# sarpel/wakeword-jupyterlab

Measured on AMD Instinct MI355X. Metric: 1s/16kHz clips/sec end-to-end (mel+CNN+LSTM), higher is better.
Workload: dtype f32 in/out/accumulate; conv and LSTM-gate GEMM products as f16x3 split (3 f16 MFMAs per fp32 product block, ~2^-21 rel.)

## Files before the change

### wakeword-jupyterlab_amd/csrc/ww_logmel.hip

```cpp
#include <mutex>
#include <type_traits>

#include "ww_internal.h"

namespace ww {

constexpr int kSlab = 2048 + 4;
constexpr int kPartialInSlab = 1032;
static_assert(kPartialInSlab + kPieces <= kSlab, "piece sums must fit behind the power spectrum");

template <int WAVES, int FR = kFrames>
struct K1Layout {
    static constexpr int kWaves = WAVES;
    static constexpr int kThreads = WAVES * 64;
    static constexpr int kMelStr = FR + 1;
    static constexpr int kOffMel = WAVES * kSlab;
    static constexpr int kOffRed = kOffMel + kMels * kMelStr;
    static constexpr int kOffFrm = kOffRed + 16;
    static constexpr int kOffInvw = kOffFrm + WAVES * FR;
    static constexpr int kOffFlag = kOffInvw + kMels;
    static constexpr int kOffDcNy = kOffFlag + 4;
    static constexpr int kOffPinfo = kOffDcNy + FR;
    static constexpr int kOffFp0 = kOffPinfo + kPieces;
    static constexpr int kOffFcnt = kOffFp0 + kMels;
    static constexpr int kOffTw2 = kOffFcnt + kMels;
    static constexpr int kOffTwp = kOffTw2 + 7 * 16 * 2;
    static constexpr int kLdsFloats = kOffTwp + 512 * 2;
    static constexpr int kWavesPerSimd = WAVES == 4 ? (FR != kFrames ? 2 : 3) : 2;
    static constexpr int kBlocksPerCu = WAVES == 4 ? (FR != kFrames ? 2 : 3) : 1;
    static_assert(kOffPinfo % 4 == 0 && kOffTw2 % 4 == 0 && kOffTwp % 2 == 0, "LDS table alignment");
    static_assert(FR % WAVES == 0 && WAVES <= 8, "frames are dealt to the waves in whole rounds; red[] holds 16 floats");
    static_assert(FR == kFrames || FR == 64, "the long-clip tile: 64 frames, frames dealt round-robin");
    static_assert(kBlocksPerCu * sizeof(float) * kLdsFloats <= 160 * 1024, "LDS per CU");
};

__device__ __forceinline__ float2 operator+(float2 a, float2 b) { return make_float2(a.x + b.x, a.y + b.y); }
__device__ __forceinline__ float2 operator-(float2 a, float2 b) { return make_float2(a.x - b.x, a.y - b.y); }
__device__ __forceinline__ float2 cmul(float2 a, float2 b) {
    return make_float2(fmaf(a.x, b.x, -a.y * b.y), fmaf(a.x, b.y, a.y * b.x));
}
__device__ __forceinline__ float2 mul_neg_i(float2 a) { return make_float2(a.y, -a.x); }

__device__ __forceinline__ void dft4(float2& a0, float2& a1, float2& a2, float2& a3) {
    const float2 t0 = a0 + a2, t1 = a0 - a2, t2 = a1 + a3, t3 = mul_neg_i(a1 - a3);
    a0 = t0 + t2; a2 = t0 - t2; a1 = t1 + t3; a3 = t1 - t3;
}

__device__ __forceinline__ void dft8(float2 (&v)[8]) {
    constexpr float c = 0.70710678118654752440f;
    float2 e0 = v[0], e1 = v[2], e2 = v[4], e3 = v[6];
    float2 o0 = v[1], o1 = v[3], o2 = v[5], o3 = v[7];
    dft4(e0, e1, e2, e3);
    dft4(o0, o1, o2, o3);
    o1 = make_float2(c * (o1.x + o1.y), c * (o1.y - o1.x));
    o2 = mul_neg_i(o2);
    o3 = make_float2(c * (o3.y - o3.x), -c * (o3.x + o3.y));
    v[0] = e0 + o0; v[4] = e0 - o0;
    v[1] = e1 + o1; v[5] = e1 - o1;
    v[2] = e2 + o2; v[6] = e2 - o2;
    v[3] = e3 + o3; v[7] = e3 - o3;
}

__device__ __forceinline__ void dft16(float2 (&v)[16]) {
    float2 e[8], o[8];
#pragma unroll
    for (int i = 0; i < 8; ++i) { e[i] = v[2 * i]; o[i] = v[2 * i + 1]; }
    dft8(e);
    dft8(o);
    constexpr float c1 = 0.92387953251128675613f, s1 = 0.38268343236508977173f;
    constexpr float c2 = 0.70710678118654752440f;
    const float2 w[8] = {{1.f, 0.f}, {c1, -s1}, {c2, -c2}, {s1, -c1}, {0.f, -1.f}, {-s1, -c1}, {-c2, -c2}, {-c1, -s1}};
#pragma unroll
    for (int k = 0; k < 8; ++k) {
        const float2 t = (k == 0) ? o[0] : (k == 4 ? mul_neg_i(o[4]) : cmul(o[k], w[k]));
        v[k] = e[k] + t;
        v[k + 8] = e[k] - t;
    }
}

__device__ __forceinline__ float db10(float x) {
#pragma clang fp contract(off)
    return 10.0f * log10f(x);
}

__device__ __forceinline__ void lds_order() {
    __builtin_amdgcn_fence(__ATOMIC_RELEASE, "wavefront");
    __builtin_amdgcn_wave_barrier();
    __builtin_amdgcn_fence(__ATOMIC_ACQUIRE, "wavefront");
}

__device__ __forceinline__ float absmax3(float a, float b, float m) {
    float r;
    asm("v_max3_f32 %0, |%1|, |%2|, %3" : "=v"(r) : "v"(a), "v"(b), "v"(m));
    return r;
}

using u32x4_t = __attribute__((ext_vector_type(4))) unsigned int;

template <bool RING>
__device__ __forceinline__ void load_frame(float4 (&sn)[8], __amdgpu_buffer_rsrc_t rsrc, int base, int ring_pos, int ring_len) {
#pragma unroll
    for (int n1 = 0; n1 < 8; ++n1) {
        const int idx = base + 256 * n1;
        int off = idx * 4;
        if constexpr (RING) {
            int at = idx + ring_pos;
            at = at >= ring_len ? at - ring_len : at;
            off = (idx >= 0 && idx < ring_len) ? at * 4 : -1;
        }
        const u32x4_t v = __builtin_amdgcn_raw_buffer_load_b128(rsrc, off, 0, 0);
        sn[n1] = __builtin_bit_cast(float4, v);
    }
}

constexpr uint32_t kRedoMark = 0x7fc5a11eu;
constexpr float kFloorRatio = 1.0e-5f;

#ifdef WW_STAMPS
__device__ unsigned long long g_stamps[16];
#define STAMP(i) do { unsigned long long t__; asm volatile("s_memtime %0\n\ts_waitcnt lgkmcnt(0)" : "=s"(t__) :: "memory"); \
    if (stamp_on) { acc_st[i] += t__ - last_st; } last_st = t__; } while (0)
#else
#define STAMP(i) do {} while (0)
#endif

template <bool RING, int WAVES, int FR = kFrames>
__global__ __launch_bounds__(WAVES * 64, (K1Layout<WAVES, FR>::kWavesPerSimd)) void logmel_kernel(const float* __restrict__ pcm, int64_t clip_stride,
                                                             int clip_len, int n_clips, int normalize,
                                                             const int32_t* __restrict__ ring_pos_p, int ring_len,
                                                             const LogmelTables* __restrict__ tb,
                                                             float* __restrict__ out, int mark, int n_frames) {
    using L = K1Layout<WAVES, FR>;
    constexpr int kMelStride = L::kMelStr;
    const int nfr = FR == kFrames ? kFrames : n_frames;
    constexpr int kWavesPerBlock = WAVES, kThreads = L::kThreads;
    constexpr int kOffMel = L::kOffMel, kOffRed = L::kOffRed, kOffFrm = L::kOffFrm, kOffInvw = L::kOffInvw, kOffFlag = L::kOffFlag,
                  kOffDcNy = L::kOffDcNy, kOffPinfo = L::kOffPinfo, kOffFp0 = L::kOffFp0,
                  kOffFcnt = L::kOffFcnt, kOffTw2 = L::kOffTw2, kOffTwp = L::kOffTwp;
    extern __shared__ __attribute__((aligned(16))) float lds[];
    float* mel = lds + kOffMel;
    float* red = lds + kOffRed;
    const float4* pw4 = reinterpret_cast<const float4*>(&tb->piece_w[0][0][0]);
    const int* pinfo = reinterpret_cast<const int*>(lds + kOffPinfo);
    const int* fp0 = reinterpret_cast<const int*>(lds + kOffFp0);
    const int* fcnt = reinterpret_cast<const int*>(lds + kOffFcnt);
    const float4* tw2_4 = reinterpret_cast<const float4*>(lds + kOffTw2);
    const float2* twp_2 = reinterpret_cast<const float2*>(lds + kOffTwp);

    const int tid = threadIdx.x;
    const int lane_id = tid & 63;
    const int lane = lane_id;
    const int wave = __builtin_amdgcn_readfirstlane(tid >> 6);
    float* slab = lds + wave * kSlab;
    float2* slab2 = reinterpret_cast<float2*>(slab);
    float4* slab4 = reinterpret_cast<float4*>(slab);
    float* partial = slab + kPartialInSlab;
    const float4* tw1_4 = reinterpret_cast<const float4*>(&tb->tw1[0][0]);
    const float4* win4 = reinterpret_cast<const float4*>(&tb->window[0]);

    for (int i = tid; i < kPieces; i += kThreads) reinterpret_cast<int*>(lds)[kOffPinfo + i] = tb->piece_info[i];
    if (tid < kMels) {
        reinterpret_cast<int*>(lds)[kOffFp0 + tid] = tb->filt_p0[tid];
        reinterpret_cast<int*>(lds)[kOffFcnt + tid] = tb->filt_cnt[tid];
        lds[kOffInvw + tid] = tb->band_bins[tid];
    }
    if (tid < 4) reinterpret_cast<uint32_t*>(lds)[kOffFlag + tid] = 0u;
    for (int i = tid; i < 7 * 16 * 2; i += kThreads) lds[kOffTw2 + i] = (&tb->tw2[0][0].x)[i];
    for (int i = tid; i < 512 * 2; i += kThreads) lds[kOffTwp + i] = (&tb->twp[0].x)[i];
    const int ring_pos = RING ? *ring_pos_p : 0;
    __syncthreads();
    const int my_p0a = fp0[lane], my_cnta = fcnt[lane];
    const int my_p0b = lane + 64 < kMels ? fp0[lane + 64] : 0, my_cntb = lane + 64 < kMels ? fcnt[lane + 64] : 0;

#ifdef WW_STAMPS
    const bool stamp_on = true;
    unsigned long long acc_st[10] = {0, 0, 0, 0, 0, 0, 0, 0, 0, 0}, last_st = 0;
    STAMP(9);
#endif

    const unsigned clip_bytes = unsigned(clip_len) * 4u;
    auto clip_rsrc = [&](int c) {
        const bool ok = c < n_clips;
        const float* base = pcm + int64_t(ok ? c : 0) * clip_stride;
        return __builtin_amdgcn_make_buffer_rsrc(const_cast<float*>(base), 0, ok ? clip_bytes : 0u, 0x00020000);
    };
    const int kRounds = FR == kFrames ? kFrames / kWavesPerBlock : (nfr + kWavesPerBlock - 1) / kWavesPerBlock;
    const int frame0 = wave;
    float4 sn[8];
    load_frame<RING>(sn, clip_rsrc(blockIdx.x), frame0 * kHop - kNfft / 2 + 4 * lane, ring_pos, ring_len);
    int clip_it = 0;
#pragma unroll 1
    for (int clip = blockIdx.x; clip < n_clips; clip += gridDim.x, ++clip_it) {
        const __amdgpu_buffer_rsrc_t rs_cur = clip_rsrc(clip), rs_next = clip_rsrc(clip + int(gridDim.x));
        float peak = 0.f;

#pragma unroll 1
        for (int round = 0; round < kRounds; ++round) {
            const int frame = round * kWavesPerBlock + wave;
            int lane = lane_id;
            asm volatile("" : "+v"(lane));
            const int k1r = lane >> 3, jr = lane & 7;
            const int base_next = (frame + kWavesPerBlock) * kHop - kNfft / 2 + 4 * lane;

            STAMP(8);
            float2 za[8], zb[8];
#pragma unroll
            for (int n1 = 0; n1 < 8; ++n1) {
                const float4 s = sn[n1];
                const float4 w = win4[64 * n1 + lane];
                if (n1 == 4 || n1 == 5) peak = absmax3(s.z, s.w, absmax3(s.x, s.y, peak));
                za[n1] = make_float2(s.x * w.x, s.y * w.y);
                zb[n1] = make_float2(s.z * w.z, s.w * w.w);
            }
            float4 t1[7];
#pragma unroll
            for (int k1 = 1; k1 < 8; ++k1) t1[k1 - 1] = tw1_4[(k1 - 1) * 64 + lane];
            __builtin_amdgcn_sched_barrier(0);
            dft8(za);
            dft8(zb);
            slab4[lane] = make_float4(za[0].x, za[0].y, zb[0].x, zb[0].y);
#pragma unroll
            for (int k1 = 1; k1 < 8; ++k1) {
                const float4 t = t1[k1 - 1];
                const float2 a = cmul(za[k1], make_float2(t.x, t.y));
                const float2 b = cmul(zb[k1], make_float2(t.z, t.w));
                slab4[k1 * 64 + (lane ^ (8 * ((k1 >> 1) & 1)))] = make_float4(a.x, a.y, b.x, b.y);
            }
            lds_order();
            STAMP(0);
            {
                const int s8 = 8 * ((k1r >> 1) & 1);
                const float4* x1e = slab4 + k1r * 64 + jr + s8;
                const float4* x1o = slab4 + k1r * 64 + jr - s8;
#pragma unroll
                for (int n2 = 0; n2 < 8; ++n2) {
                    const float4 v = (n2 & 1) ? x1o[n2 * 8] : x1e[n2 * 8];
                    za[n2] = make_float2(v.x, v.y);
                    zb[n2] = make_float2(v.z, v.w);
                }
                float4 t2[7];
#pragma unroll
                for (int k2 = 1; k2 < 8; ++k2) t2[k2 - 1] = tw2_4[(k2 - 1) * 8 + jr];
                lds_order();
                __builtin_amdgcn_sched_barrier(0);
                dft8(za);
                dft8(zb);
                float4* x2w[4];
#pragma unroll
                for (int hk = 0; hk < 4; ++hk) x2w[hk] = slab4 + 64 * k1r + (jr ^ (4 * (k1r & 1) + hk));
#pragma unroll
                for (int k2 = 0; k2 < 8; ++k2) {
                    float2 a = za[k2], b = zb[k2];
                    if (k2 > 0) {
                        const float4 t = t2[k2 - 1];
                        a = cmul(a, make_float2(t.x, t.y));
                        b = cmul(b, make_float2(t.z, t.w));
                    }
                    x2w[k2 >> 1][8 * k2] = make_float4(a.x, a.y, b.x, b.y);
                }
            }
            lds_order();
            STAMP(1);
            {
                float2 u[16];
                const int sw2 = (lane >> 1) & 7;
#pragma unroll
                for (int m = 0; m < 8; ++m) {
                    const float4 v = slab4[lane * 8 + (m ^ sw2)];
                    u[2 * m] = make_float2(v.x, v.y);
                    u[2 * m + 1] = make_float2(v.z, v.w);
                }
                lds_order();
                dft16(u);
                const int lp = (lane >> 3) + 8 * (lane & 7);
                float2* zw = slab2 + (lp ^ (((lp >> 4) & 3) << 1));
#pragma unroll
                for (int kk = 0; kk < 16; ++kk) zw[64 * kk] = u[kk];
            }
            lds_order();
            STAMP(2);
            float4 pw0[kPieceRounds], pw1[kPieceRounds];
#pragma unroll
            for (int c = 0; c < kPieceRounds; ++c) {
                pw0[c] = pw4[c * kPieceSlots + lane];
                pw1[c] = pw4[kPieces + c * kPieceSlots + lane];
            }
            {
                const bool last = round + 1 == kRounds;
                load_frame<RING>(sn, last ? rs_next : rs_cur, last ? frame0 * kHop - kNfft / 2 + 4 * lane : base_next, ring_pos,
                                 ring_len);
            }
            {
                float2 a[8], b[8];
                const int lowb = (64 - lane) & 63;
                const float2* za_p = slab2 + (lane ^ (((lane >> 4) & 3) << 1));
                const float2* zb_p = slab2 + (lowb ^ (((lowb >> 4) & 3) << 1)) + (lane == 0 ? 64 : 0);
#pragma unroll
                for (int j = 0; j < 8; ++j) {
                    a[j] = za_p[64 * j];
                    b[j] = zb_p[64 * (15 - j)];
                }
                if (lane == 0) {
                    if (mark) lds[kOffDcNy + frame] = 2.0f * fmaf(a[0].x, a[0].x, a[0].y * a[0].y);
                    a[0] = slab2[512];
                    b[0] = a[0];
                }
                float2 twj[8];
#pragma unroll
                for (int j = 0; j < 8; ++j) twj[j] = twp_2[lane + 64 * j];
                lds_order();
                __builtin_amdgcn_sched_barrier(0);
#pragma unroll
                for (int j = 0; j < 8; ++j) {
                    const int k = (j == 0 && lane == 0) ? 512 : lane + 64 * j;
                    const float2 tw = twj[j];
                    const float2 e = make_float2(0.5f * (a[j].x + b[j].x), 0.5f * (a[j].y - b[j].y));
                    const float2 o = make_float2(0.5f * (a[j].y + b[j].y), 0.5f * (b[j].x - a[j].x));
                    const float2 t = cmul(o, tw);
                    const float2 p = e + t, m = e - t;
                    slab[k] = fmaf(p.x, p.x, p.y * p.y);
                    slab[1024 - k] = fmaf(m.x, m.x, m.y * m.y);
                }
                if (lane == 0) slab[0] = 0.f;
            }
            lds_order();
            STAMP(3);
            {
                int info[kPieceRounds];
                float4 s0[kPieceRounds], s1[kPieceRounds];
#pragma unroll
                for (int c = 0; c < kPieceRounds; ++c) info[c] = pinfo[c * kPieceSlots + lane];
#pragma unroll
                for (int c = 0; c < kPieceRounds; ++c) {
                    const float4* s4 = reinterpret_cast<const float4*>(slab + (info[c] & 0xffff));
                    s0[c] = s4[0];
                    s1[c] = s4[1];
                }
                __builtin_amdgcn_sched_barrier(0);
#pragma unroll
                for (int c = 0; c < kPieceRounds; ++c) {
                    const float4 w0 = pw0[c], w1 = pw1[c];
                    float acc = w0.x * s0[c].x;
                    acc = fmaf(w0.y, s0[c].y, acc);
                    acc = fmaf(w0.z, s0[c].z, acc);
                    acc = fmaf(w0.w, s0[c].w, acc);
                    acc = fmaf(w1.x, s1[c].x, acc);
                    acc = fmaf(w1.y, s1[c].y, acc);
                    acc = fmaf(w1.z, s1[c].z, acc);
                    acc = fmaf(w1.w, s1[c].w, acc);
                    partial[info[c] >> 16] = acc;
                }
                lds_order();
                STAMP(4);
#pragma unroll
                for (int pass = 0; pass < 2; ++pass) {
                    const int f = lane + 64 * pass;
                    const int p0 = pass ? my_p0b : my_p0a, cnt = pass ? my_cntb : my_cnta;
                    if (f < kMels) {
                        float v[10];
#pragma unroll
                        for (int q = 0; q < 10; ++q) v[q] = partial[p0 + (q < cnt ? q : 0)];
                        float acc = 0.f;
#pragma unroll
                        for (int q = 0; q < 10; ++q) acc += (q < cnt) ? v[q] : 0.f;
                        mel[f * kMelStride + frame] = acc;
                    }
                }
            }
            lds_order();
            STAMP(5);
        }
        if constexpr (FR != kFrames) {
            __syncthreads();
            uint32_t* flag = reinterpret_cast<uint32_t*>(lds) + kOffFlag;
            if (mark && tid == 0) { flag[2 * ((clip_it + 1) & 1)] = 0u; flag[2 * ((clip_it + 1) & 1) + 1] = 0u; }
            const bool fr_live = lane < nfr;
            const float* invw = lds + kOffInvw;
            float* frm = lds + kOffFrm;
            float mmax = 0.f, e_part = 0.f;
            if (fr_live)
                for (int b = wave; b < kMels; b += kWavesPerBlock) {
                    const float p = mel[b * kMelStride + lane];
                    mmax = fmaxf(mmax, p);
                    if (mark) e_part = fmaf(p, invw[b], e_part);
                }
            if (mark) frm[wave * FR + lane] = e_part;
#pragma unroll
            for (int off = 32; off > 0; off >>= 1) {
                mmax = fmaxf(mmax, __shfl_xor(mmax, off));
                peak = fmaxf(peak, __shfl_xor(peak, off));
            }
            if (lane == 0) { red[wave] = mmax; red[kWavesPerBlock + wave] = peak; }
            __syncthreads();
            mmax = red[0];
            peak = red[kWavesPerBlock];
#pragma unroll
            for (int w = 1; w < kWavesPerBlock; ++w) { mmax = fmaxf(mmax, red[w]); peak = fmaxf(peak, red[kWavesPerBlock + w]); }
            const float amin = 1e-10f;
            float g2 = 1.f;
            if (normalize) { const float g = 1.0f / peak; g2 = g * g; }
            float ref = mmax * g2;
            ref = ref < amin ? amin : ref;
            const float ref_db = db10(ref);
            float* __restrict__ o = out + int64_t(clip) * (kMels * nfr);
            float floor_e = 0.f;
            if (mark) {
#pragma unroll
                for (int w = 0; w < kWavesPerBlock; ++w) floor_e += frm[w * FR + lane];
                floor_e += lds[kOffDcNy + lane];
                floor_e *= kFloorRatio;
            }
            const float live_thr = fmaxf(mmax * 0.99e-8f, amin / g2);
            bool redo = false;
            if (fr_live)
                for (int b = wave; b < kMels; b += kWavesPerBlock) {
                    const float p = mel[b * kMelStride + lane];
                    float v = p * g2;
                    v = v < amin ? amin : v;
                    float db = db10(v) - ref_db;
                    db = db < -80.0f ? -80.0f : db;
                    o[b * nfr + lane] = db;
                    if (mark) redo |= p > live_thr && p * invw[b] < floor_e;
                }
            if (mark) {
                const unsigned long long bal = __builtin_amdgcn_ballot_w64(redo);
                if (bal != 0ull && lane == 0) {
                    __hip_atomic_fetch_or(flag + 2 * (clip_it & 1), uint32_t(bal), __ATOMIC_RELAXED, __HIP_MEMORY_SCOPE_WORKGROUP);
                    __hip_atomic_fetch_or(flag + 2 * (clip_it & 1) + 1, uint32_t(bal >> 32), __ATOMIC_RELAXED, __HIP_MEMORY_SCOPE_WORKGROUP);
                }
            }
            __syncthreads();
            if (mark) {
                const uint32_t f_lo = flag[2 * (clip_it & 1)], f_hi = flag[2 * (clip_it & 1) + 1];
                if ((f_lo | f_hi) != 0u) {
                    if (fr_live)
                        for (int b = wave; b < kMels; b += kWavesPerBlock)
                            if (b * nfr + lane >= 3) o[b * nfr + lane] = mel[b * kMelStride + lane] * g2;
                    if (tid == 0) {
                        reinterpret_cast<uint32_t*>(o)[0] = kRedoMark;
                        reinterpret_cast<uint32_t*>(o)[1] = f_lo | 7u;
                        reinterpret_cast<uint32_t*>(o)[2] = f_hi;
                    }
                    __syncthreads();
                }
            }
        } else {
        __syncthreads();
        STAMP(6);
        uint32_t* flag = reinterpret_cast<uint32_t*>(lds) + kOffFlag;
        if (mark && tid == 0) flag[(clip_it + 1) & 1] = 0u;

        float mmax = 0.f, e_part = 0.f;
        const float* invw = lds + kOffInvw;
        float* frm = lds + kOffFrm;
        for (int idx = tid; idx < kMels * kFrames; idx += kThreads) {
            const float p = mel[(idx >> 5) * kMelStride + (idx & 31)];
            mmax = fmaxf(mmax, p);
            if (mark) e_part = fmaf(p, invw[idx >> 5], e_part);
        }
        if (mark) {
            e_part += __shfl_xor(e_part, 32);
            if (lane < 32) frm[wave * 32 + lane] = e_part;
        }
#pragma unroll
        for (int off = 32; off > 0; off >>= 1) {
            mmax = fmaxf(mmax, __shfl_xor(mmax, off));
            peak = fmaxf(peak, __shfl_xor(peak, off));
        }
        if (lane == 0) { red[wave] = mmax; red[kWavesPerBlock + wave] = peak; }
        __syncthreads();
        mmax = red[0];
        peak = red[kWavesPerBlock];
#pragma unroll
        for (int w = 1; w < kWavesPerBlock; ++w) { mmax = fmaxf(mmax, red[w]); peak = fmaxf(peak, red[kWavesPerBlock + w]); }

        const float amin = 1e-10f;
        float g2 = 1.f;
        if (normalize) { const float g = 1.0f / peak; g2 = g * g; }
        float ref = mmax * g2;
        ref = ref < amin ? amin : ref;
        const float ref_db = db10(ref);
        float* __restrict__ o = out + int64_t(clip) * (kMels * kFrames);
        float floor_e = 0.f;
        if (mark) {
#pragma unroll
            for (int w = 0; w < kWavesPerBlock; ++w) floor_e += frm[w * 32 + (tid & 31)];
            floor_e += lds[kOffDcNy + (tid & 31)];
            floor_e *= kFloorRatio;
        }
        const float live_thr = fmaxf(mmax * 0.99e-8f, amin / g2);
        bool redo = false;
        for (int idx = tid; idx < kMels * kFrames; idx += kThreads) {
            const float p = mel[(idx >> 5) * kMelStride + (idx & 31)];
            float v = p * g2;
            v = v < amin ? amin : v;
            float db = db10(v) - ref_db;
            db = db < -80.0f ? -80.0f : db;
            o[idx] = db;
            if (mark) redo |= p > live_thr && p * invw[idx >> 5] < floor_e;
        }
        if (mark) {
            const unsigned long long bal = __builtin_amdgcn_ballot_w64(redo);
            const uint32_t fm = uint32_t(bal) | uint32_t(bal >> 32);
            if (fm != 0u && lane == 0) __hip_atomic_fetch_or(flag + (clip_it & 1), fm, __ATOMIC_RELAXED, __HIP_MEMORY_SCOPE_WORKGROUP);
        }
        __syncthreads();
        if (mark) {
            const uint32_t fm = flag[clip_it & 1];
            if (fm != 0u) {
                for (int idx = tid; idx < kMels * kFrames; idx += kThreads)
                    if (idx >= 2) o[idx] = mel[(idx >> 5) * kMelStride + (idx & 31)] * g2;
                if (tid == 0) {
                    reinterpret_cast<uint32_t*>(o)[0] = kRedoMark;
                    reinterpret_cast<uint32_t*>(o)[1] = fm | 3u;
                }
            }
        }
        }
        STAMP(7);
    }
#ifdef WW_STAMPS
    if (lane == 0 && wave == 1 && blockIdx.x == 7)
        for (int i = 0; i < 10; ++i) atomicAdd(&g_stamps[i], acc_st[i]);
#endif
}
#ifdef WW_STAMPS
extern "C" __attribute__((visibility("default"))) int ww_debug_stamps(unsigned long long* out) {
    unsigned long long z[16] = {};
    if (hipMemcpyFromSymbol(out, HIP_SYMBOL(g_stamps), sizeof(z)) != hipSuccess) return -1;
    (void)hipMemcpyToSymbol(HIP_SYMBOL(g_stamps), z, sizeof(z));
    return 0;
}
#endif

struct cd { double x, y; };
struct alignas(16) cd2 { cd a, b; };
__device__ __forceinline__ cd operator+(cd a, cd b) { return {a.x + b.x, a.y + b.y}; }
__device__ __forceinline__ cd operator-(cd a, cd b) { return {a.x - b.x, a.y - b.y}; }
__device__ __forceinline__ cd cmul(cd a, cd b) { return {fma(a.x, b.x, -a.y * b.y), fma(a.x, b.y, a.y * b.x)}; }
__device__ __forceinline__ cd mul_neg_i(cd a) { return {a.y, -a.x}; }
__device__ __forceinline__ void dft4(cd& a0, cd& a1, cd& a2, cd& a3) {
    const cd t0 = a0 + a2, t1 = a0 - a2, t2 = a1 + a3, t3 = mul_neg_i(a1 - a3);
    a0 = t0 + t2; a2 = t0 - t2; a1 = t1 + t3; a3 = t1 - t3;
}
__device__ __forceinline__ void dft8(cd (&v)[8]) {
    constexpr double c = 0.70710678118654752440;
    cd e0 = v[0], e1 = v[2], e2 = v[4], e3 = v[6];
    cd o0 = v[1], o1 = v[3], o2 = v[5], o3 = v[7];
    dft4(e0, e1, e2, e3);
    dft4(o0, o1, o2, o3);
    o1 = {c * (o1.x + o1.y), c * (o1.y - o1.x)};
    o2 = mul_neg_i(o2);
    o3 = {c * (o3.y - o3.x), -c * (o3.x + o3.y)};
    v[0] = e0 + o0; v[4] = e0 - o0;
    v[1] = e1 + o1; v[5] = e1 - o1;
    v[2] = e2 + o2; v[6] = e2 - o2;
    v[3] = e3 + o3; v[7] = e3 - o3;
}
__device__ __forceinline__ void dft16(cd (&v)[16]) {
    cd e[8], o[8];
#pragma unroll
    for (int i = 0; i < 8; ++i) { e[i] = v[2 * i]; o[i] = v[2 * i + 1]; }
    dft8(e);
    dft8(o);
    constexpr double c1 = 0.92387953251128675613, s1 = 0.38268343236508977173, c2 = 0.70710678118654752440;
    const cd w[8] = {{1., 0.}, {c1, -s1}, {c2, -c2}, {s1, -c1}, {0., -1.}, {-s1, -c1}, {-c2, -c2}, {-c1, -s1}};
#pragma unroll
    for (int k = 0; k < 8; ++k) {
        const cd t = (k == 0) ? o[0] : (k == 4 ? mul_neg_i(o[4]) : cmul(o[k], w[k]));
        v[k] = e[k] + t;
        v[k + 8] = e[k] - t;
    }
}

constexpr int kSlab64 = 2 * 2048 + 8;
template <int FR = kFrames>
struct K64Layout {
    static constexpr int kMelStr = FR + 1;
    static constexpr int kOffMel = 4 * kSlab64;
    static constexpr int kOffRed = kOffMel + kMels * kMelStr;
    static constexpr int kOffPinfo = kOffRed + 16;
    static constexpr int kOffFp0 = kOffPinfo + kPieces;
    static constexpr int kOffFcnt = kOffFp0 + kMels;
    static constexpr int kOffTw2 = (kOffFcnt + kMels + 3) & ~3;
    static constexpr int kLdsFloats = kOffTw2 + 7 * 16 * 4;
    static constexpr int kBlocksPerCu = FR == kFrames ? 2 : 1;
    static_assert(kOffMel % 4 == 0 && kOffTw2 % 4 == 0, "16-byte alignment of the double tables");
    static_assert(kBlocksPerCu * (sizeof(float) * kLdsFloats + 512) <= 160 * 1024, "LDS per CU");
};
constexpr int k64LdsFloats = K64Layout<>::kLdsFloats;
static_assert(sizeof(float) * k64LdsFloats + 512 <= 80 * 1024, "two logmel64 workgroups per CU");

template <bool RING, bool ONLY_FLAGGED, int FR = kFrames>
__global__ __launch_bounds__(256, 2) void logmel64_kernel(const float* __restrict__ pcm, int64_t clip_stride, int clip_len, int n_clips,
                                                          int normalize, const int32_t* __restrict__ ring_pos_p, int ring_len,
                                                          const LogmelTables* __restrict__ tb, float* __restrict__ out, int n_frames) {
    constexpr int kWavesPerBlock = 4, kThreads = 256;
    using L64 = K64Layout<FR>;
    constexpr int kMelStride = L64::kMelStr, k64OffMel = L64::kOffMel, k64OffRed = L64::kOffRed, k64OffPinfo = L64::kOffPinfo,
                  k64OffFp0 = L64::kOffFp0, k64OffFcnt = L64::kOffFcnt, k64OffTw2 = L64::kOffTw2;
    const int nfr = FR == kFrames ? kFrames : n_frames;
    using mask_t = typename std::conditional<FR == kFrames, uint32_t, unsigned long long>::type;
    extern __shared__ __attribute__((aligned(16))) float lds[];
    float* mel = lds + k64OffMel;
    float* red = lds + k64OffRed;
    const int* pinfo = reinterpret_cast<const int*>(lds + k64OffPinfo);
    const int* fp0 = reinterpret_cast<const int*>(lds + k64OffFp0);
    const int* fcnt = reinterpret_cast<const int*>(lds + k64OffFcnt);
    const cd2* tw2_u = reinterpret_cast<const cd2*>(lds + k64OffTw2);
    const cd* twp_c = reinterpret_cast<const cd*>(&tb->twp_d[0]);
    const float4* pw4 = reinterpret_cast<const float4*>(&tb->piece_w[0][0][0]);
    const cd2* tw1_u = reinterpret_cast<const cd2*>(&tb->tw1_d[0][0]);
    const double* win = &tb->window_d[0];

    const int tid = threadIdx.x, lane_id = tid & 63, lane = lane_id;
    const int wave = __builtin_amdgcn_readfirstlane(tid >> 6);
    if constexpr (ONLY_FLAGGED) {
        int any = 0;
        for (int c = int(blockIdx.x) + tid * int(gridDim.x); c < n_clips; c += kThreads * int(gridDim.x))
            any |= __float_as_uint(__builtin_nontemporal_load(out + int64_t(c) * (kMels * nfr))) == kRedoMark;
        if (!__syncthreads_or(any)) return;
    }
    float* slabf = lds + wave * kSlab64;
    cd* slabc = reinterpret_cast<cd*>(slabf);
    cd* slabA = slabc;
    cd* slabB = slabc + 512;
    float* partial = slabf + kPartialInSlab;

    for (int i = tid; i < kPieces; i += kThreads) reinterpret_cast<int*>(lds)[k64OffPinfo + i] = tb->piece_info[i];
    if (tid < kMels) {
        reinterpret_cast<int*>(lds)[k64OffFp0 + tid] = tb->filt_p0[tid];
        reinterpret_cast<int*>(lds)[k64OffFcnt + tid] = tb->filt_cnt[tid];
    }
    for (int i = tid; i < 7 * 16 * 2; i += kThreads) reinterpret_cast<double*>(lds + k64OffTw2)[i] = (&tb->tw2_d[0][0].x)[i];
    const int ring_pos = RING ? *ring_pos_p : 0;
    __syncthreads();
    const int my_p0a = fp0[lane], my_cnta = fcnt[lane];
    const int my_p0b = lane + 64 < kMels ? fp0[lane + 64] : 0, my_cntb = lane + 64 < kMels ? fcnt[lane + 64] : 0;
    const unsigned clip_bytes = unsigned(clip_len) * 4u;

#pragma unroll 1
    for (int clip = blockIdx.x; clip < n_clips; clip += gridDim.x) {
        float* __restrict__ o = out + int64_t(clip) * (kMels * nfr);
        mask_t fmask = FR == kFrames ? mask_t(0xffffffffu) : (nfr >= 64 ? ~mask_t(0) : (mask_t(1) << nfr) - 1u);
        if constexpr (ONLY_FLAGGED) {
            if (__builtin_amdgcn_readfirstlane(__float_as_uint(__builtin_nontemporal_load(o))) != kRedoMark) continue;
            fmask = __builtin_amdgcn_readfirstlane(__float_as_uint(__builtin_nontemporal_load(o + 1)));
            if constexpr (FR != kFrames)
                fmask |= mask_t(__builtin_amdgcn_readfirstlane(__float_as_uint(__builtin_nontemporal_load(o + 2)))) << 32;
            for (int idx = tid; idx < kMels * nfr; idx += kThreads) {
                const int b = FR == kFrames ? idx >> 5 : idx / nfr, t = FR == kFrames ? idx & 31 : idx - b * nfr;
                if (!((fmask >> t) & 1u)) mel[b * kMelStride + t] = __builtin_nontemporal_load(o + idx);
            }
        }
        const int n_mine = (int(FR == kFrames ? __builtin_popcount(uint32_t(fmask)) : __builtin_popcountll(fmask)) - wave + kWavesPerBlock - 1) /
                           kWavesPerBlock;
        auto nth_frame = [&](int n) -> int {
            mask_t m = fmask;
            for (int i = 0; i < n && m; ++i) m &= m - 1u;
            return m ? (FR == kFrames ? __builtin_ctz(uint32_t(m)) : __builtin_ctzll(m)) : 2 * FR;
        };
        const __amdgpu_buffer_rsrc_t rs = __builtin_amdgcn_make_buffer_rsrc(const_cast<float*>(pcm + int64_t(clip) * clip_stride), 0,
                                                                             clip_bytes, 0x00020000);
        float peak = 0.f;
        if (normalize) {
#pragma unroll 1
            for (int round = 0; round < (nfr + kWavesPerBlock - 1) / kWavesPerBlock; ++round) {
                float4 sn[8];
                load_frame<RING>(sn, rs, (round * kWavesPerBlock + wave) * kHop - kNfft / 2 + 4 * lane, ring_pos, ring_len);
                peak = absmax3(sn[4].z, sn[4].w, absmax3(sn[4].x, sn[4].y, peak));
                peak = absmax3(sn[5].z, sn[5].w, absmax3(sn[5].x, sn[5].y, peak));
            }
#pragma unroll
            for (int off = 32; off > 0; off >>= 1) peak = fmaxf(peak, __shfl_xor(peak, off));
            if (lane == 0) red[wave] = peak;
            __syncthreads();
            peak = fmaxf(fmaxf(red[0], red[1]), fmaxf(red[2], red[3]));
            __syncthreads();
        }
        float4 sn[8];
        int frame = nth_frame(wave);
        load_frame<RING>(sn, rs, frame * kHop - kNfft / 2 + 4 * lane, ring_pos, ring_len);
#pragma unroll 1
        for (int round = 0; round < n_mine; ++round) {
            const int frame_next = nth_frame((round + 1) * kWavesPerBlock + wave);
            int lane = lane_id;
            asm volatile("" : "+v"(lane));
            const int k1r = lane >> 3, jr = lane & 7;
            cd za[8], zb[8];
#pragma unroll
            for (int n1 = 0; n1 < 8; ++n1) {
                float4 s = sn[n1];
                if (normalize) { s.x = __fdiv_rn(s.x, peak); s.y = __fdiv_rn(s.y, peak); s.z = __fdiv_rn(s.z, peak); s.w = __fdiv_rn(s.w, peak); }
                const double* w = win + 4 * (64 * n1 + lane);
                za[n1] = {double(s.x) * w[0], double(s.y) * w[1]};
                zb[n1] = {double(s.z) * w[2], double(s.w) * w[3]};
            }
            dft8(za);
            dft8(zb);
            slabA[lane] = za[0];
            slabB[lane] = zb[0];
#pragma unroll
            for (int k1 = 1; k1 < 8; ++k1) {
                const cd2 t = tw1_u[(k1 - 1) * 64 + lane];
                const int at = k1 * 64 + (lane ^ (8 * ((k1 >> 1) & 1)));
                slabA[at] = cmul(za[k1], t.a);
                slabB[at] = cmul(zb[k1], t.b);
            }
            lds_order();
            load_frame<RING>(sn, rs, frame_next * kHop - kNfft / 2 + 4 * lane, ring_pos, ring_len);
            {
                const int s8 = 8 * ((k1r >> 1) & 1);
                const cd* x1e = slabA + k1r * 64 + jr + s8;
                const cd* x1o = slabA + k1r * 64 + jr - s8;
#pragma unroll
                for (int n2 = 0; n2 < 8; ++n2) {
                    const cd* src = (n2 & 1) ? x1o + n2 * 8 : x1e + n2 * 8;
                    za[n2] = src[0];
                    zb[n2] = src[512];
                }
                lds_order();
                dft8(za);
                dft8(zb);
                cd* x2w[4];
#pragma unroll
                for (int hk = 0; hk < 4; ++hk) x2w[hk] = slabA + 64 * k1r + (jr ^ (4 * (k1r & 1) + hk));
#pragma unroll
                for (int k2 = 0; k2 < 8; ++k2) {
                    cd a = za[k2], b = zb[k2];
                    if (k2 > 0) {
                        const cd2 t = tw2_u[(k2 - 1) * 8 + jr];
                        a = cmul(a, t.a);
                        b = cmul(b, t.b);
                    }
                    x2w[k2 >> 1][8 * k2] = a;
                    x2w[k2 >> 1][8 * k2 + 512] = b;
                }
            }
            lds_order();
            {
                cd u[16];
                const int sw2 = (lane >> 1) & 7;
#pragma unroll
                for (int m = 0; m < 8; ++m) {
                    const cd* src = slabA + lane * 8 + (m ^ sw2);
                    u[2 * m] = src[0];
                    u[2 * m + 1] = src[512];
                }
                lds_order();
                dft16(u);
                const int lp = (lane >> 3) + 8 * (lane & 7);
                cd* zw = slabc + (lp ^ ((lp >> 3) & 7));
#pragma unroll
                for (int kk = 0; kk < 16; ++kk) zw[64 * kk] = u[kk];
            }
            lds_order();
            {
                cd a[8], b[8];
                const int lowb = (64 - lane) & 63;
                const cd* za_p = slabc + (lane ^ ((lane >> 3) & 7));
                const cd* zb_p = slabc + (lowb ^ ((lowb >> 3) & 7)) + (lane == 0 ? 64 : 0);
#pragma unroll
                for (int j = 0; j < 8; ++j) {
                    a[j] = za_p[64 * j];
                    b[j] = zb_p[64 * (15 - j)];
                }
                if (lane == 0) { a[0] = slabc[512]; b[0] = a[0]; }
                lds_order();
#pragma unroll
                for (int j = 0; j < 8; ++j) {
                    const int k = (j == 0 && lane == 0) ? 512 : lane + 64 * j;
                    const cd tw = twp_c[lane + 64 * j];
                    const cd e = {0.5 * (a[j].x + b[j].x), 0.5 * (a[j].y - b[j].y)};
                    const cd od = {0.5 * (a[j].y + b[j].y), 0.5 * (b[j].x - a[j].x)};
                    const cd t = cmul(od, tw);
                    const float px = float(e.x + t.x), py = float(e.y + t.y), mx = float(e.x - t.x), my = float(e.y - t.y);
                    slabf[k] = fmaf(px, px, py * py);
                    slabf[1024 - k] = fmaf(mx, mx, my * my);
                }
                if (lane == 0) slabf[0] = 0.f;
            }
            lds_order();
            {
                int info[kPieceRounds];
                float4 s0[kPieceRounds], s1[kPieceRounds], pw0[kPieceRounds], pw1[kPieceRounds];
#pragma unroll
                for (int c = 0; c < kPieceRounds; ++c) {
                    info[c] = pinfo[c * kPieceSlots + lane];
                    pw0[c] = pw4[c * kPieceSlots + lane];
                    pw1[c] = pw4[kPieces + c * kPieceSlots + lane];
                }
#pragma unroll
                for (int c = 0; c < kPieceRounds; ++c) {
                    const float4* s4 = reinterpret_cast<const float4*>(slabf + (info[c] & 0xffff));
                    s0[c] = s4[0];
                    s1[c] = s4[1];
                }
#pragma unroll
                for (int c = 0; c < kPieceRounds; ++c) {
                    const float4 w0 = pw0[c], w1 = pw1[c];
                    float acc = w0.x * s0[c].x;
                    acc = fmaf(w0.y, s0[c].y, acc);
                    acc = fmaf(w0.z, s0[c].z, acc);
                    acc = fmaf(w0.w, s0[c].w, acc);
                    acc = fmaf(w1.x, s1[c].x, acc);
                    acc = fmaf(w1.y, s1[c].y, acc);
                    acc = fmaf(w1.z, s1[c].z, acc);
                    acc = fmaf(w1.w, s1[c].w, acc);
                    partial[info[c] >> 16] = acc;
                }
                lds_order();
#pragma unroll
                for (int pass = 0; pass < 2; ++pass) {
                    const int f = lane + 64 * pass;
                    const int p0 = pass ? my_p0b : my_p0a, cnt = pass ? my_cntb : my_cnta;
                    if (f < kMels) {
                        float acc = 0.f;
                        for (int q = 0; q < cnt; ++q) acc += partial[p0 + q];
                        mel[f * kMelStride + frame] = acc;
                    }
                }
            }
            lds_order();
            frame = frame_next;
        }
        __syncthreads();
        float mmax = 0.f;
        bool any_nan = false;
        for (int idx = tid; idx < kMels * nfr; idx += kThreads) {
            const int b = FR == kFrames ? idx >> 5 : idx / nfr, t = FR == kFrames ? idx & 31 : idx - b * nfr;
            const float p = mel[b * kMelStride + t];
            any_nan |= p != p;
            mmax = fmaxf(mmax, p);
        }
#pragma unroll
        for (int off = 32; off > 0; off >>= 1) mmax = fmaxf(mmax, __shfl_xor(mmax, off));
        any_nan = __builtin_amdgcn_ballot_w64(any_nan) != 0ull;
        if (lane == 0) red[wave] = any_nan ? __uint_as_float(0x7fc00000u) : mmax;
        __syncthreads();
        mmax = red[0];
#pragma unroll
        for (int w = 1; w < kWavesPerBlock; ++w) mmax = (red[w] != red[w] || mmax != mmax) ? __uint_as_float(0x7fc00000u) : fmaxf(mmax, red[w]);
        const float amin = 1e-10f;
        float ref = mmax;
        ref = ref < amin ? amin : ref;
        const float ref_db = db10(ref);
        for (int idx = tid; idx < kMels * nfr; idx += kThreads) {
            const int b = FR == kFrames ? idx >> 5 : idx / nfr, t = FR == kFrames ? idx & 31 : idx - b * nfr;
            float v = mel[b * kMelStride + t];
            v = v < amin ? amin : v;
            float db = db10(v) - ref_db;
            db = db < -80.0f ? -80.0f : db;
            o[idx] = db;
        }
        __syncthreads();
    }
}

template <int WAVES, int FR = kFrames>
static int launch_logmel_w(const float* pcm, int64_t n_clips, int64_t clip_stride, int64_t clip_len, int normalize,
                           const int32_t* ring_pos, int64_t ring_len, float* logmel, const LogmelTables* tb, int mark, hipStream_t stream,
                           int n_frames = kFrames) {
    using L = K1Layout<WAVES, FR>;
    const int64_t resident = int64_t(device_cu_count()) * L::kBlocksPerCu;
    const int grid = int(n_clips < resident ? n_clips : resident);
    const size_t lds_bytes = sizeof(float) * L::kLdsFloats;
    if (ring_pos)
        hipLaunchKernelGGL((logmel_kernel<true, WAVES, FR>), dim3(grid), dim3(L::kThreads), lds_bytes, stream, pcm, clip_stride, int(clip_len),
                           int(n_clips), normalize, ring_pos, int(ring_len), tb, logmel, mark, n_frames);
    else
        hipLaunchKernelGGL((logmel_kernel<false, WAVES, FR>), dim3(grid), dim3(L::kThreads), lds_bytes, stream, pcm, clip_stride, int(clip_len),
                           int(n_clips), normalize, ring_pos, int(ring_len), tb, logmel, mark, n_frames);
    WW_HIP(hipGetLastError());
    return WW_OK;
}

template <bool ONLY_FLAGGED, int FR = kFrames>
static int launch_logmel64(const float* pcm, int64_t n_clips, int64_t clip_stride, int64_t clip_len, int normalize,
                           const int32_t* ring_pos, int64_t ring_len, float* logmel, const LogmelTables* tb, hipStream_t stream,
                           int n_frames = kFrames) {
    const int64_t resident = K64Layout<FR>::kBlocksPerCu * int64_t(device_cu_count());
    const int grid = int(n_clips < resident ? n_clips : resident);
    const size_t lds_bytes = sizeof(float) * K64Layout<FR>::kLdsFloats;
    if (ring_pos)
        hipLaunchKernelGGL((logmel64_kernel<true, ONLY_FLAGGED, FR>), dim3(grid), dim3(256), lds_bytes, stream, pcm, clip_stride, int(clip_len),
                           int(n_clips), normalize, ring_pos, int(ring_len), tb, logmel, n_frames);
    else
        hipLaunchKernelGGL((logmel64_kernel<false, ONLY_FLAGGED, FR>), dim3(grid), dim3(256), lds_bytes, stream, pcm, clip_stride, int(clip_len),
                           int(n_clips), normalize, ring_pos, int(ring_len), tb, logmel, n_frames);
    WW_HIP(hipGetLastError());
    return WW_OK;
}

static int logmel_opt_in_lds() {
    static std::mutex mu;
    static bool done[64] = {};
    std::lock_guard<std::mutex> lock(mu);
    int dev = 0;
    WW_HIP(hipGetDevice(&dev));
    if (dev < 0 || dev >= 64) return fail(WW_EINVAL, "device ordinal out of range");
    if (done[dev]) return WW_OK;
    const int b4 = int(sizeof(float) * K1Layout<4>::kLdsFloats), b8 = int(sizeof(float) * K1Layout<8>::kLdsFloats);
    const int b64 = int(sizeof(float) * k64LdsFloats);
    WW_HIP(hipFuncSetAttribute(reinterpret_cast<const void*>(logmel_kernel<true, 4>), hipFuncAttributeMaxDynamicSharedMemorySize, b4));
    WW_HIP(hipFuncSetAttribute(reinterpret_cast<const void*>(logmel_kernel<false, 4>), hipFuncAttributeMaxDynamicSharedMemorySize, b4));
    WW_HIP(hipFuncSetAttribute(reinterpret_cast<const void*>(logmel_kernel<true, 8>), hipFuncAttributeMaxDynamicSharedMemorySize, b8));
    WW_HIP(hipFuncSetAttribute(reinterpret_cast<const void*>(logmel_kernel<false, 8>), hipFuncAttributeMaxDynamicSharedMemorySize, b8));
    WW_HIP(hipFuncSetAttribute(reinterpret_cast<const void*>(logmel64_kernel<true, true>), hipFuncAttributeMaxDynamicSharedMemorySize, b64));
    WW_HIP(hipFuncSetAttribute(reinterpret_cast<const void*>(logmel64_kernel<true, false>), hipFuncAttributeMaxDynamicSharedMemorySize, b64));
    WW_HIP(hipFuncSetAttribute(reinterpret_cast<const void*>(logmel64_kernel<false, true>), hipFuncAttributeMaxDynamicSharedMemorySize, b64));
    WW_HIP(hipFuncSetAttribute(reinterpret_cast<const void*>(logmel64_kernel<false, false>), hipFuncAttributeMaxDynamicSharedMemorySize, b64));
    const int c4 = int(sizeof(float) * K1Layout<4, 64>::kLdsFloats), c8 = int(sizeof(float) * K1Layout<8, 64>::kLdsFloats);
    const int c64 = int(sizeof(float) * K64Layout<64>::kLdsFloats);
    WW_HIP(hipFuncSetAttribute(reinterpret_cast<const void*>(logmel_kernel<true, 4, 64>), hipFuncAttributeMaxDynamicSharedMemorySize, c4));
    WW_HIP(hipFuncSetAttribute(reinterpret_cast<const void*>(logmel_kernel<false, 4, 64>), hipFuncAttributeMaxDynamicSharedMemorySize, c4));
    WW_HIP(hipFuncSetAttribute(reinterpret_cast<const void*>(logmel_kernel<true, 8, 64>), hipFuncAttributeMaxDynamicSharedMemorySize, c8));
    WW_HIP(hipFuncSetAttribute(reinterpret_cast<const void*>(logmel_kernel<false, 8, 64>), hipFuncAttributeMaxDynamicSharedMemorySize, c8));
    WW_HIP(hipFuncSetAttribute(reinterpret_cast<const void*>(logmel64_kernel<true, true, 64>), hipFuncAttributeMaxDynamicSharedMemorySize, c64));
    WW_HIP(hipFuncSetAttribute(reinterpret_cast<const void*>(logmel64_kernel<true, false, 64>), hipFuncAttributeMaxDynamicSharedMemorySize, c64));
    WW_HIP(hipFuncSetAttribute(reinterpret_cast<const void*>(logmel64_kernel<false, true, 64>), hipFuncAttributeMaxDynamicSharedMemorySize, c64));
    WW_HIP(hipFuncSetAttribute(reinterpret_cast<const void*>(logmel64_kernel<false, false, 64>), hipFuncAttributeMaxDynamicSharedMemorySize, c64));
    done[dev] = true;
    return WW_OK;
}

int launch_logmel(const float* pcm, int64_t n_clips, int64_t clip_stride, int64_t clip_len, int normalize,
                  const int32_t* ring_pos, int64_t ring_len, float* logmel, hipStream_t stream) {
    if (n_clips == 0) return WW_OK;
    const LogmelTables* tb = device_tables();
    if (!tb) return WW_EHIP;
    if (int rc = logmel_opt_in_lds()) return rc;
    const int mode = logmel_math_mode();
    if (mode == WW_LOGMEL_MATH_F64)
        return launch_logmel64<false>(pcm, n_clips, clip_stride, clip_len, normalize, ring_pos, ring_len, logmel, tb, stream);
    const int mark = mode == WW_LOGMEL_MATH_AUTO;
    int rc;
    if (n_clips <= device_cu_count())
        rc = launch_logmel_w<8>(pcm, n_clips, clip_stride, clip_len, normalize, ring_pos, ring_len, logmel, tb, mark, stream);
    else
        rc = launch_logmel_w<4>(pcm, n_clips, clip_stride, clip_len, normalize, ring_pos, ring_len, logmel, tb, mark, stream);
    if (rc != WW_OK || !mark) return rc;
    return launch_logmel64<true>(pcm, n_clips, clip_stride, clip_len, normalize, ring_pos, ring_len, logmel, tb, stream);
}

int launch_logmel_frames(const float* pcm, int64_t n_clips, int64_t clip_stride, int64_t clip_len, int64_t n_samples, int normalize,
                         const int32_t* ring_pos, int64_t ring_len, float* logmel, hipStream_t stream) {
    const int T = int(1 + n_samples / kHop);
    if (T == kFrames) return launch_logmel(pcm, n_clips, clip_stride, clip_len, normalize, ring_pos, ring_len, logmel, stream);
    if (n_clips == 0) return WW_OK;
    const LogmelTables* tb = device_tables();
    if (!tb) return WW_EHIP;
    if (int rc = logmel_opt_in_lds()) return rc;
    const int mode = logmel_math_mode();
    if (mode == WW_LOGMEL_MATH_F64)
        return launch_logmel64<false, 64>(pcm, n_clips, clip_stride, clip_len, normalize, ring_pos, ring_len, logmel, tb, stream, T);
    const int mark = mode == WW_LOGMEL_MATH_AUTO;
    int rc;
    if (n_clips <= device_cu_count())
        rc = launch_logmel_w<8, 64>(pcm, n_clips, clip_stride, clip_len, normalize, ring_pos, ring_len, logmel, tb, mark, stream, T);
    else
        rc = launch_logmel_w<4, 64>(pcm, n_clips, clip_stride, clip_len, normalize, ring_pos, ring_len, logmel, tb, mark, stream, T);
    if (rc != WW_OK || !mark) return rc;
    return launch_logmel64<true, 64>(pcm, n_clips, clip_stride, clip_len, normalize, ring_pos, ring_len, logmel, tb, stream, T);
}
int launch_logmel_frames(const float* pcm, int64_t n_clips, int64_t clip_stride, int64_t clip_len, int64_t n_samples, int normalize,
                         float* logmel, hipStream_t stream) {
    return launch_logmel_frames(pcm, n_clips, clip_stride, clip_len, n_samples, normalize, nullptr, 0, logmel, stream);
}

}
```

Before: 4.839 million.

## Pack three clips per 12-wave logmel workgroup and cache window/twiddles in LDS

For large batches, the log-mel kernel now runs one 12-wave workgroup per CU holding three independent 4-wave clip slots, instead of three separate 4-wave blocks. Each slot gets its own mel tile, reduction, flag and DC/Nyquist regions, while the filter and twiddle tables are loaded into LDS once and shared by all three slots. The window and tw1 tables also move from global memory into LDS, aiming to cut global/L2 table traffic and duplicated table setup. The cost is that the slots now share workgroup-wide barriers, so one slot's stalls hold up the others, and a partial last group needs clip_live guards and a combined redo flag.

```diff
diff --git a/wakeword-jupyterlab_amd/csrc/ww_logmel.hip b/wakeword-jupyterlab_amd/csrc/ww_logmel.hip
--- a/wakeword-jupyterlab_amd/csrc/ww_logmel.hip
+++ b/wakeword-jupyterlab_amd/csrc/ww_logmel.hip
@@ -13,26 +13,36 @@
 struct K1Layout {
     static constexpr int kWaves = WAVES;
     static constexpr int kThreads = WAVES * 64;
+    static constexpr int kSlots = WAVES == 12 ? 3 : 1;
+    static constexpr int kSlotWaves = WAVES / kSlots;
+    static constexpr int kSlotThreads = kSlotWaves * 64;
+    static constexpr bool kTablesInLds = WAVES == 12;
     static constexpr int kMelStr = FR + 1;
+    static constexpr int kMelTile = kMels * kMelStr;
     static constexpr int kOffMel = WAVES * kSlab;
-    static constexpr int kOffRed = kOffMel + kMels * kMelStr;
-    static constexpr int kOffFrm = kOffRed + 16;
+    static constexpr int kOffRed = kOffMel + kSlots * kMelTile;
+    static constexpr int kOffFrm = kOffRed + kSlots * 16;
     static constexpr int kOffInvw = kOffFrm + WAVES * FR;
     static constexpr int kOffFlag = kOffInvw + kMels;
-    static constexpr int kOffDcNy = kOffFlag + 4;
-    static constexpr int kOffPinfo = kOffDcNy + FR;
+    static constexpr int kOffDcNy = kOffFlag + kSlots * 4;
+    static constexpr int kOffPinfo = kOffDcNy + kSlots * FR;
     static constexpr int kOffFp0 = kOffPinfo + kPieces;
     static constexpr int kOffFcnt = kOffFp0 + kMels;
     static constexpr int kOffTw2 = kOffFcnt + kMels;
     static constexpr int kOffTwp = kOffTw2 + 7 * 16 * 2;
-    static constexpr int kLdsFloats = kOffTwp + 512 * 2;
-    static constexpr int kWavesPerSimd = WAVES == 4 ? (FR != kFrames ? 2 : 3) : 2;
+    static constexpr int kOffWin = kOffTwp + 512 * 2;
+    static constexpr int kOffTw1 = kOffWin + (kTablesInLds ? kNfft : 0);
+    static constexpr int kLdsFloats = kOffTw1 + (kTablesInLds ? 7 * 64 * 4 : 0);
+    static constexpr int kWavesPerSimd = WAVES == 12 ? 3 : (WAVES == 4 ? (FR != kFrames ? 2 : 3) : 2);
     static constexpr int kBlocksPerCu = WAVES == 4 ? (FR != kFrames ? 2 : 3) : 1;
-    static_assert(kOffPinfo % 4 == 0 && kOffTw2 % 4 == 0 && kOffTwp % 2 == 0, "LDS table alignment");
-    static_assert(FR % WAVES == 0 && WAVES <= 8, "frames are dealt to the waves in whole rounds; red[] holds 16 floats");
+    static_assert(kOffMel % 4 == 0 && kOffPinfo % 4 == 0 && kOffTw2 % 4 == 0 && kOffTwp % 2 == 0 && kOffWin % 4 == 0 && kOffTw1 % 4 == 0,
+                  "LDS table alignment");
+    static_assert(FR % kSlotWaves == 0 && kSlotWaves <= 8, "frames are dealt to a slot's waves in whole rounds; red[] holds 16 floats per slot");
+    static_assert(kSlots == 1 || (FR == kFrames && kSlotWaves == 4), "the lock-step form: three 1 s clips, four waves each");
     static_assert(FR == kFrames || FR == 64, "the long-clip tile: 64 frames, frames dealt round-robin");
     static_assert(kBlocksPerCu * sizeof(float) * kLdsFloats <= 160 * 1024, "LDS per CU");
 };
+static_assert(sizeof(float) * K1Layout<12>::kLdsFloats <= 152 * 1024, "the 12-wave form's LDS map");
 
 __device__ __forceinline__ float2 operator+(float2 a, float2 b) { return make_float2(a.x + b.x, a.y + b.y); }
 __device__ __forceinline__ float2 operator-(float2 a, float2 b) { return make_float2(a.x - b.x, a.y - b.y); }
@@ -133,13 +143,11 @@
     using L = K1Layout<WAVES, FR>;
     constexpr int kMelStride = L::kMelStr;
     const int nfr = FR == kFrames ? kFrames : n_frames;
-    constexpr int kWavesPerBlock = WAVES, kThreads = L::kThreads;
+    constexpr int kWavesPerBlock = L::kSlotWaves, kThreads = L::kSlotThreads, kSlots = L::kSlots;
     constexpr int kOffMel = L::kOffMel, kOffRed = L::kOffRed, kOffFrm = L::kOffFrm, kOffInvw = L::kOffInvw, kOffFlag = L::kOffFlag,
                   kOffDcNy = L::kOffDcNy, kOffPinfo = L::kOffPinfo, kOffFp0 = L::kOffFp0,
                   kOffFcnt = L::kOffFcnt, kOffTw2 = L::kOffTw2, kOffTwp = L::kOffTwp;
     extern __shared__ __attribute__((aligned(16))) float lds[];
-    float* mel = lds + kOffMel;
-    float* red = lds + kOffRed;
     const float4* pw4 = reinterpret_cast<const float4*>(&tb->piece_w[0][0][0]);
     const int* pinfo = reinterpret_cast<const int*>(lds + kOffPinfo);
     const int* fp0 = reinterpret_cast<const int*>(lds + kOffFp0);
@@ -147,26 +155,40 @@
     const float4* tw2_4 = reinterpret_cast<const float4*>(lds + kOffTw2);
     const float2* twp_2 = reinterpret_cast<const float2*>(lds + kOffTwp);
 
-    const int tid = threadIdx.x;
-    const int lane_id = tid & 63;
+    const int lane_id = threadIdx.x & 63;
     const int lane = lane_id;
-    const int wave = __builtin_amdgcn_readfirstlane(tid >> 6);
-    float* slab = lds + wave * kSlab;
+    const int wave_wg = __builtin_amdgcn_readfirstlane(threadIdx.x >> 6);
+    const int slot = kSlots == 1 ? 0 : wave_wg / kWavesPerBlock;
+    const int wave = wave_wg - slot * kWavesPerBlock;
+    const int tid = wave * 64 + lane_id;
+    float* mel = lds + kOffMel + slot * L::kMelTile;
+    float* red = lds + kOffRed + slot * 16;
+    float* slab = lds + wave_wg * kSlab;
     float2* slab2 = reinterpret_cast<float2*>(slab);
     float4* slab4 = reinterpret_cast<float4*>(slab);
     float* partial = slab + kPartialInSlab;
-    const float4* tw1_4 = reinterpret_cast<const float4*>(&tb->tw1[0][0]);
-    const float4* win4 = reinterpret_cast<const float4*>(&tb->window[0]);
-
-    for (int i = tid; i < kPieces; i += kThreads) reinterpret_cast<int*>(lds)[kOffPinfo + i] = tb->piece_info[i];
-    if (tid < kMels) {
-        reinterpret_cast<int*>(lds)[kOffFp0 + tid] = tb->filt_p0[tid];
-        reinterpret_cast<int*>(lds)[kOffFcnt + tid] = tb->filt_cnt[tid];
-        lds[kOffInvw + tid] = tb->band_bins[tid];
+    const float4* tw1_4 = L::kTablesInLds ? reinterpret_cast<const float4*>(lds + L::kOffTw1) : reinterpret_cast<const float4*>(&tb->tw1[0][0]);
+    const float4* win4 = L::kTablesInLds ? reinterpret_cast<const float4*>(lds + L::kOffWin) : reinterpret_cast<const float4*>(&tb->window[0]);
+
+    {
+        const int wtid = threadIdx.x;
+        constexpr int kWgThreads = L::kThreads;
+        for (int i = wtid; i < kPieces; i += kWgThreads) reinterpret_cast<int*>(lds)[kOffPinfo + i] = tb->piece_info[i];
+        if (wtid < kMels) {
+            reinterpret_cast<int*>(lds)[kOffFp0 + wtid] = tb->filt_p0[wtid];
+            reinterpret_cast<int*>(lds)[kOffFcnt + wtid] = tb->filt_cnt[wtid];
+            lds[kOffInvw + wtid] = tb->band_bins[wtid];
+        }
+        if (wtid < 4 * kSlots) reinterpret_cast<uint32_t*>(lds)[kOffFlag + wtid] = 0u;
+        for (int i = wtid; i < 7 * 16 * 2; i += kWgThreads) lds[kOffTw2 + i] = (&tb->tw2[0][0].x)[i];
+        for (int i = wtid; i < 512 * 2; i += kWgThreads) lds[kOffTwp + i] = (&tb->twp[0].x)[i];
+        if constexpr (L::kTablesInLds) {
+            float4* wl = reinterpret_cast<float4*>(lds + L::kOffWin);
+            float4* tl = reinterpret_cast<float4*>(lds + L::kOffTw1);
+            for (int i = wtid; i < kNfft / 4; i += kWgThreads) wl[i] = reinterpret_cast<const float4*>(&tb->window[0])[i];
+            for (int i = wtid; i < 7 * 64; i += kWgThreads) tl[i] = reinterpret_cast<const float4*>(&tb->tw1[0][0])[i];
+        }
     }
-    if (tid < 4) reinterpret_cast<uint32_t*>(lds)[kOffFlag + tid] = 0u;
-    for (int i = tid; i < 7 * 16 * 2; i += kThreads) lds[kOffTw2 + i] = (&tb->tw2[0][0].x)[i];
-    for (int i = tid; i < 512 * 2; i += kThreads) lds[kOffTwp + i] = (&tb->twp[0].x)[i];
     const int ring_pos = RING ? *ring_pos_p : 0;
     __syncthreads();
     const int my_p0a = fp0[lane], my_cnta = fcnt[lane];
@@ -187,11 +209,13 @@
     const int kRounds = FR == kFrames ? kFrames / kWavesPerBlock : (nfr + kWavesPerBlock - 1) / kWavesPerBlock;
     const int frame0 = wave;
     float4 sn[8];
-    load_frame<RING>(sn, clip_rsrc(blockIdx.x), frame0 * kHop - kNfft / 2 + 4 * lane, ring_pos, ring_len);
+    load_frame<RING>(sn, clip_rsrc(int(blockIdx.x) * kSlots + slot), frame0 * kHop - kNfft / 2 + 4 * lane, ring_pos, ring_len);
     int clip_it = 0;
 #pragma unroll 1
-    for (int clip = blockIdx.x; clip < n_clips; clip += gridDim.x, ++clip_it) {
-        const __amdgpu_buffer_rsrc_t rs_cur = clip_rsrc(clip), rs_next = clip_rsrc(clip + int(gridDim.x));
+    for (int grp = blockIdx.x; grp * kSlots < n_clips; grp += gridDim.x, ++clip_it) {
+        const int clip = grp * kSlots + slot;
+        const bool clip_live = kSlots == 1 || clip < n_clips;
+        const __amdgpu_buffer_rsrc_t rs_cur = clip_rsrc(clip), rs_next = clip_rsrc(clip + int(gridDim.x) * kSlots);
         float peak = 0.f;
 
 #pragma unroll 1
@@ -301,7 +325,7 @@
                     b[j] = zb_p[64 * (15 - j)];
                 }
                 if (lane == 0) {
-                    if (mark) lds[kOffDcNy + frame] = 2.0f * fmaf(a[0].x, a[0].x, a[0].y * a[0].y);
+                    if (mark) lds[kOffDcNy + slot * FR + frame] = 2.0f * fmaf(a[0].x, a[0].x, a[0].y * a[0].y);
                     a[0] = slab2[512];
                     b[0] = a[0];
                 }
@@ -447,12 +471,12 @@
         } else {
         __syncthreads();
         STAMP(6);
-        uint32_t* flag = reinterpret_cast<uint32_t*>(lds) + kOffFlag;
+        uint32_t* flag = reinterpret_cast<uint32_t*>(lds) + kOffFlag + slot * 4;
         if (mark && tid == 0) flag[(clip_it + 1) & 1] = 0u;
 
         float mmax = 0.f, e_part = 0.f;
         const float* invw = lds + kOffInvw;
-        float* frm = lds + kOffFrm;
+        float* frm = lds + kOffFrm + slot * (kWavesPerBlock * 32);
         for (int idx = tid; idx < kMels * kFrames; idx += kThreads) {
             const float p = mel[(idx >> 5) * kMelStride + (idx & 31)];
             mmax = fmaxf(mmax, p);
@@ -485,7 +509,7 @@
         if (mark) {
 #pragma unroll
             for (int w = 0; w < kWavesPerBlock; ++w) floor_e += frm[w * 32 + (tid & 31)];
-            floor_e += lds[kOffDcNy + (tid & 31)];
+            floor_e += lds[kOffDcNy + slot * 32 + (tid & 31)];
             floor_e *= kFloorRatio;
         }
         const float live_thr = fmaxf(mmax * 0.99e-8f, amin / g2);
@@ -496,7 +520,7 @@
             v = v < amin ? amin : v;
             float db = db10(v) - ref_db;
             db = db < -80.0f ? -80.0f : db;
-            o[idx] = db;
+            if (clip_live) o[idx] = db;
             if (mark) redo |= p > live_thr && p * invw[idx >> 5] < floor_e;
         }
         if (mark) {
@@ -507,13 +531,22 @@
         __syncthreads();
         if (mark) {
             const uint32_t fm = flag[clip_it & 1];
-            if (fm != 0u) {
-                for (int idx = tid; idx < kMels * kFrames; idx += kThreads)
-                    if (idx >= 2) o[idx] = mel[(idx >> 5) * kMelStride + (idx & 31)] * g2;
-                if (tid == 0) {
-                    reinterpret_cast<uint32_t*>(o)[0] = kRedoMark;
-                    reinterpret_cast<uint32_t*>(o)[1] = fm | 3u;
-                }
+            uint32_t any = fm;
+            if constexpr (kSlots > 1) {
+                any = 0u;
+#pragma unroll
+                for (int sl = 0; sl < kSlots; ++sl) any |= reinterpret_cast<const uint32_t*>(lds)[kOffFlag + sl * 4 + (clip_it & 1)];
+            }
+            if (any != 0u) {
+                if (fm != 0u && clip_live) {
+                    for (int idx = tid; idx < kMels * kFrames; idx += kThreads)
+                        if (idx >= 2) o[idx] = mel[(idx >> 5) * kMelStride + (idx & 31)] * g2;
+                    if (tid == 0) {
+                        reinterpret_cast<uint32_t*>(o)[0] = kRedoMark;
+                        reinterpret_cast<uint32_t*>(o)[1] = fm | 3u;
+                    }
+                }
+                __syncthreads();
             }
         }
         }
@@ -863,7 +896,8 @@
                            int n_frames = kFrames) {
     using L = K1Layout<WAVES, FR>;
     const int64_t resident = int64_t(device_cu_count()) * L::kBlocksPerCu;
-    const int grid = int(n_clips < resident ? n_clips : resident);
+    const int64_t groups = (n_clips + L::kSlots - 1) / L::kSlots;
+    const int grid = int(groups < resident ? groups : resident);
     const size_t lds_bytes = sizeof(float) * L::kLdsFloats;
     if (ring_pos)
         hipLaunchKernelGGL((logmel_kernel<true, WAVES, FR>), dim3(grid), dim3(L::kThreads), lds_bytes, stream, pcm, clip_stride, int(clip_len),
@@ -900,10 +934,10 @@
     WW_HIP(hipGetDevice(&dev));
     if (dev < 0 || dev >= 64) return fail(WW_EINVAL, "device ordinal out of range");
     if (done[dev]) return WW_OK;
-    const int b4 = int(sizeof(float) * K1Layout<4>::kLdsFloats), b8 = int(sizeof(float) * K1Layout<8>::kLdsFloats);
+    const int b12 = int(sizeof(float) * K1Layout<12>::kLdsFloats), b8 = int(sizeof(float) * K1Layout<8>::kLdsFloats);
     const int b64 = int(sizeof(float) * k64LdsFloats);
-    WW_HIP(hipFuncSetAttribute(reinterpret_cast<const void*>(logmel_kernel<true, 4>), hipFuncAttributeMaxDynamicSharedMemorySize, b4));
-    WW_HIP(hipFuncSetAttribute(reinterpret_cast<const void*>(logmel_kernel<false, 4>), hipFuncAttributeMaxDynamicSharedMemorySize, b4));
+    WW_HIP(hipFuncSetAttribute(reinterpret_cast<const void*>(logmel_kernel<true, 12>), hipFuncAttributeMaxDynamicSharedMemorySize, b12));
+    WW_HIP(hipFuncSetAttribute(reinterpret_cast<const void*>(logmel_kernel<false, 12>), hipFuncAttributeMaxDynamicSharedMemorySize, b12));
     WW_HIP(hipFuncSetAttribute(reinterpret_cast<const void*>(logmel_kernel<true, 8>), hipFuncAttributeMaxDynamicSharedMemorySize, b8));
     WW_HIP(hipFuncSetAttribute(reinterpret_cast<const void*>(logmel_kernel<false, 8>), hipFuncAttributeMaxDynamicSharedMemorySize, b8));
     WW_HIP(hipFuncSetAttribute(reinterpret_cast<const void*>(logmel64_kernel<true, true>), hipFuncAttributeMaxDynamicSharedMemorySize, b64));
@@ -938,7 +972,7 @@
     if (n_clips <= device_cu_count())
         rc = launch_logmel_w<8>(pcm, n_clips, clip_stride, clip_len, normalize, ring_pos, ring_len, logmel, tb, mark, stream);
     else
-        rc = launch_logmel_w<4>(pcm, n_clips, clip_stride, clip_len, normalize, ring_pos, ring_len, logmel, tb, mark, stream);
+        rc = launch_logmel_w<12>(pcm, n_clips, clip_stride, clip_len, normalize, ring_pos, ring_len, logmel, tb, mark, stream);
     if (rc != WW_OK || !mark) return rc;
     return launch_logmel64<true>(pcm, n_clips, clip_stride, clip_len, normalize, ring_pos, ring_len, logmel, tb, stream);
 }
```

Result: slower. 4.686 million (-3.2%).
